# BloodAxe/segmentation-networks-benchmark

Hardware: AMD Instinct MI355X
Metric: images/sec/GPU (fwd+bwd) ZF_UNET 224x224 bs=32; 1/2/4/8-GPU scaling (higher is better)
Workload: dtype bf16; 1 GPU; ZF_UNET 224x224 bf16 bs=32/GPU, bce_dice, SGD lr 1e-3, Dropout2d 0.2, train step torch_train.py:180-190 (configs[1]); global_batch=32, parallelism=dp1

## Files before the change

segmentation-networks-benchmark_amd/csrc/common.h:

```cpp
#pragma once
#include <hip/hip_runtime.h>
#include <hip/hip_ext.h>
#include <stdint.h>
#include <stdio.h>
#include <string.h>

#include "../../include/segnb_hip.h"

typedef __attribute__((ext_vector_type(8))) __bf16 bf16x8_t;
typedef __attribute__((ext_vector_type(16))) float f32x16_t;

struct bf16_t {
    unsigned short bits;
};

void segnb_set_error(const char* fmt, ...);

#define SEGNB_CHECK_ARG_AS(who, cond, msg)                           \
    do {                                                             \
        if (!(cond)) {                                               \
            segnb_set_error("%s: bad argument: %s", who, msg);       \
            return SEGNB_E_BADARG;                                   \
        }                                                            \
    } while (0)
// ... 73 lines not shown
    if (plan_scope__.top && g_segnb_census_on) segnb_census(#fn);                            \
    if (plan_scope__.top && segnb_plan_recording()) segnb_plan_record_call(#fn, fn, __VA_ARGS__)
void segnb_plan_refuse(const char* why);
#define SEGNB_PLAN_REFUSE(why)                                         \
    SegnbPlanScope plan_scope__;                                       \
    if (plan_scope__.top && g_segnb_census_on) segnb_census(__func__); \
    if (plan_scope__.top && segnb_plan_recording()) segnb_plan_refuse(why)

int segnb_num_cus();
bool segnb_fprop_general_forced();
int segnb_knob_fprop_dma();
int segnb_knob_fprop_dma_cfg();
int segnb_knob_fprop_dma_dbg();
int segnb_knob_fprop_nostats();
int segnb_knob_rw_store_waves();
int segnb_knob_bnreduce_fused();
int segnb_knob_fprop_deepk();
int segnb_knob_fprop_thin();
enum segnb_try_outcome {
    SEGNB_TRY_DECLINED = 0,
    SEGNB_TRY_LAUNCHED,
    SEGNB_TRY_DELIVERED,
};
inline int segnb_try_launched(segnb_try_outcome* did, int rc) {
    if (rc == 0) *did = SEGNB_TRY_LAUNCHED;
    return rc;
}
inline void segnb_kernel_took(segnb_try_outcome did, const char** served, const char* name) {
    if (did != SEGNB_TRY_DECLINED && *served == nullptr) *served = name;
}
template <class Args>
__attribute__((always_inline)) inline bool take_bn_reduce(Args& a, const segnb_conv_geom* g, const segnb_bn_reduce_epilogue* bn) {
    const long long yb = (((long long)g->N * g->Ho * g->Wo - 1) * bn->ld_y + g->Co) * 2;
    if (yb >= (1ll << 31)) return false;
    a.bn_y = (const bf16_t*)bn->y;
    a.bn_y_bytes = (unsigned)yb;
    a.bn_ld = bn->ld_y;
    a.bn_coef = bn->coef;
    a.bn_sums = bn->sums;
    a.bn_act = bn->act;
    a.bn_slope = bn->slope;
    return true;
}
template <class Args>
__attribute__((always_inline)) inline void take_act_epilogue(Args& a, const segnb_act_epilogue* ep) {
    a.ep_act = ep != nullptr ? ep->act : -1;
    a.ep_coef = ep != nullptr ? ep->coef : nullptr;
    a.ep_slope = ep != nullptr ? ep->slope : 0.f;
}
int segnb_fprop_thin_try(segnb_try_outcome* did, const segnb_conv_geom* g, const void* in, const void* wpacked, void* out,
                         hipStream_t stream, const segnb_bn_reduce_epilogue* bn);
int segnb_fprop_thin_ok(const segnb_conv_geom* g);
int segnb_knob_fprop_upd();
int segnb_knob_fprop_drop();
int segnb_knob_fprop_mask();
int segnb_fprop_dma_actmask_ok(const segnb_conv_geom* g);
int segnb_fprop_roll_actmask_ok(const segnb_conv_geom* g);
int segnb_knob_fprop_mf16();
int segnb_knob_fprop_rw();
int segnb_knob_fprop_ksplit();
float* segnb_head_scratch(size_t bytes, hipStream_t stream);
void segnb_head_bwd_finish(const float* part, int gx, int gy, int K, int C, int CT, float* dw, float* db, hipStream_t stream);
int segnb_knob_pack_blocks();
int segnb_knob_fprop_roll();
int segnb_knob_wg_cu_pct();
int segnb_knob_conv_cus();
int segnb_fprop_dma_read_stamps(unsigned long long* host_dst);
int segnb_fprop_s1_try(segnb_try_outcome* did, const segnb_conv_geom* g, const void* in, const void* wpacked, const float* bias, int bias_n,
                       void* out, double* stats, hipStream_t stream, const float* drop = nullptr, int ld_drop = 0, int stats_ld = 0);
int segnb_fprop_dma_try(segnb_try_outcome* did, const segnb_conv_geom* g, const void* in, unsigned in_bytes, const void* wpacked,
                        unsigned w_bytes, const float* bias, int bias_n, void* out, double* stats,
                        hipStream_t stream, const segnb_act_epilogue* ep = nullptr, const segnb_upcat_src* uc = nullptr,
                        const segnb_bn_reduce_epilogue* bn = nullptr);
int segnb_fprop_rw_try(segnb_try_outcome* did, const segnb_conv_geom* g, const void* in, unsigned in_bytes, const void* wpacked,
                       unsigned w_bytes, const float* bias, int bias_n, void* out, double* stats,
                       hipStream_t stream, const segnb_bn_reduce_epilogue* bn = nullptr,
                       const segnb_act_epilogue* ep = nullptr, const segnb_upcat_src* uc = nullptr,
                       const segnb_upcat_src* upsum = nullptr);
int segnb_fprop_roll_try(segnb_try_outcome* did, const segnb_conv_geom* g, const void* in, unsigned in_bytes, const void* wpacked,
                         unsigned w_bytes, const float* bias, int bias_n, void* out, double* stats, hipStream_t stream,
                         const segnb_bn_reduce_epilogue* bn = nullptr, const segnb_operand_tf* tf = nullptr,
                         const segnb_upcat_src* uc = nullptr);
int segnb_fprop_c8_try(segnb_try_outcome* did, const segnb_conv_geom* g, const void* in, const void* wpacked, const float* bias, int bias_n,
                       void* out, double* stats, hipStream_t stream, const segnb_act_epilogue* ep = nullptr);
struct segnb_wgrad_bnapply {
    const void* g;
    int ld_g;
    const void* y;
    int ld_y;
    const float* coef;
    const float* bcoef;
    int Cp;
    int act;
    float slope;
};
int segnb_wgrad_s1_try(segnb_try_outcome* did, const segnb_conv_geom* g, const void* in, const void* dout, float* dwp, int nslab,
                       hipStream_t stream, bool partial, const segnb_wgrad_bnapply* bna = nullptr,
                       const segnb_upcat_src* uc = nullptr, const segnb_wgrad_target* tgt = nullptr);
const segnb_wgrad_target* segnb_take_wgrad_target();
void segnb_wgrad_to_param(float* dwp, int Cop, int ntaps, int Cip, int nslab, const segnb_wgrad_target* tgt, bool rezero,
                          hipStream_t stream);
int segnb_wgrad_s1_slabs(const segnb_conv_geom* g);
void segnb_slab_reduce(float* dwp, long long total, int nslab, hipStream_t stream);
bool segnb_wgrad_roll_applies(const segnb_conv_geom* g);
int segnb_wgrad_roll_try(segnb_try_outcome* did, const segnb_conv_geom* g, const void* in, const void* dout, float* dwp, int nslab,
                         hipStream_t stream, bool partial, const segnb_operand_tf* tfx = nullptr, const segnb_operand_tf* tfd = nullptr);
// ... 137 lines not shown
```

segmentation-networks-benchmark_amd/csrc/fprop_dma.hip:

```cpp
#include "common.h"

#include "fprop_dma.h"

#include <mutex>
#include <vector>

#ifndef SEGNB_EXP
#define SEGNB_EXP 0
#endif

namespace {

__device__ unsigned long long g_stamps[3 * 256 * 4];
#define FD_STAMP(role, step, k)                                                                      \
    do {                                                                                            \
        if (DBG && ((a.dbg & 32) || ((a.dbg & 64) && (role) == 0 && (k) == 0)) && blockIdx.x == 0 && lane == 0 &&  \
            (step) < 256)                                                                            \
            g_stamps[((role) * 256 + (step)) * 4 + (k)] = __builtin_amdgcn_s_memtime();             \
    } while (0)

template <int BN_, int R_, int WT_, int CW_M_, bool TALL_ = false, bool MF16_ = true, int NTAP_ = 9, int UP_ = 0>
struct WsCfg {
    static constexpr bool UPD_ = UP_ == 1;
    static constexpr bool UPF = UP_ == 2;
    static_assert(UP_ == 0 || (NTAP_ == 4 && !TALL_ && MF16_), "up-sampled segment forms: 2 x 2 window, 16x16x32 form");
    static constexpr int BN = BN_, R = R_, WT = WT_;
    static constexpr int NTAP = NTAP_, KW = NTAP_ == 9 ? 3 : 2, KH = KW;
    static constexpr bool UPD = UPD_;
    static constexpr int UP = UP_;
    static constexpr int NPL = UPD_ ? 4 : 1;
    static_assert(NTAP_ == 9 || NTAP_ == 4, "3 x 3 or 2 x 2 tap window");
    static_assert(!UPD_ || (NTAP_ == 4 && !TALL_ && MF16_), "plane gather: 2 x 2 window, 16x16x32 form");
    static constexpr bool TALL = TALL_;
    static constexpr bool MF16 = MF16_;
    static constexpr int BM = TALL_ ? 256 : (R_ * WT_ + 16 * CW_M_ - 1) / (16 * CW_M_) * (16 * CW_M_);
    static constexpr int TM16 = BM / CW_M_ / 16, TN16 = BN_ / (4 / CW_M_) / 16;
    static constexpr int NB = 4;
    static constexpr int NT = 512, NCW = 4, NLW = 4;
    static_assert(R * WT <= BM, "tile pixels");
    static constexpr int NRD = TM16 + TN16, NMF = TM16 * TN16;
    static constexpr int rd_before(int q) { return (q * NRD + NMF - 1) / NMF; }
    static constexpr int WAVES_M = CW_M_, WAVES_N = NCW / CW_M_;
    static constexpr int WM = BM / WAVES_M, WN = BN / WAVES_N;
    static constexpr int TM = WM / 32, TN = WN / 32;
    static constexpr int XR = R + KH - 1, XC = WT + 2, NPIX = XR * XC;
    static constexpr int APIECES = (NPIX + 7) / 8;
    static constexpr int A_BYTES = APIECES * 1024;
    static constexpr int NBW = 2, NAW = 2;
    static constexpr int APW = (APIECES + NAW - 1) / NAW;
    static constexpr int A_STEPS = NTAP - 2;
    static constexpr int APS = (APW + A_STEPS - 1) / A_STEPS;
    static constexpr int BPIECES = BN / 8;
    static constexpr int B_STAGE = BN * 128;
    static constexpr int BPW = BPIECES / NBW;
    static constexpr int OUT_ROW = BN * 2 + 16;
    static constexpr int OC = BN / 8;
    static constexpr int MT = NCW * 64;
    static constexpr int RPT = BM / (MT / OC);
    static constexpr int OFF_B = 2 * A_BYTES;
    static constexpr int OFF_STG = OFF_B + NB * B_STAGE;
    static constexpr int OFF_DUMMY = OFF_STG + BM * OUT_ROW;
    static constexpr int OFF_PIX = OFF_DUMMY + 1024;
    static constexpr int OFF_BIAS = OFF_PIX + 4 * BM * 4;
    static constexpr int OFF_SCALE = OFF_BIAS + BN * 4;
    static constexpr int OFF_TICKET = OFF_SCALE + BN * 4;
    static constexpr int SMEM = OFF_TICKET + 16;
    static constexpr int RED_BYTES = MT * 16 * 8;
    static_assert(WM % (MF16_ ? 16 : 32) == 0 && WN % (MF16_ ? 16 : 32) == 0 && WAVES_M * WAVES_N == NCW, "wave tiling");
    static_assert(BPIECES % NBW == 0 && NBW + NAW == NLW, "fetch wave roles");
    static_assert(MT % OC == 0 && MT >= 2 * BN && RPT <= 8 && BM <= MT && BM % (MT / OC) == 0, "store pass / statistics threads");
    static constexpr bool MASK_OK = MF16_ && !TALL_ && BM == 256 && CW_M_ == 4 && SMEM + 2048 <= 160 * 1024;
    static_assert(RED_BYTES <= OFF_STG, "statistics reduction scratch");
    static_assert(SMEM <= 160 * 1024, "LDS");
    static_assert(TM + TN <= 6, "fragment wait statement");
};

template <class C, bool DBG, bool EP = false, bool STATS = true, bool SPLITK = false, bool MASK = false>
__global__ __launch_bounds__(512) void conv_fprop_ws_kernel(const FdArgs a) {
    static_assert(!SPLITK || (!EP && !DBG && C::UP == 0 && C::NTAP == 9), "split K: plain 3 x 3 forward / data gradient");
    static_assert(!MASK || (STATS && !EP && !DBG && !SPLITK && C::MF16 && C::UP == 0 && C::NTAP == 9 && !C::TALL && C::BM == 256 &&
                            C::BN == 64 && C::WAVES_M == 4 && C::SMEM + 2048 <= 160 * 1024),
                  "activation mask: plain 3 x 3 data gradient, 16x16x32 form, 256 x 64 tiles, 2 KB of mask bytes behind the LDS layout");
    constexpr int BN = C::BN, R = C::R, WT = C::WT, BM = C::BM, TM = C::TM, TN = C::TN, XC = C::XC;
    constexpr int NT = C::NT, NB = C::NB, APW = C::APW, APS = C::APS, BPW = C::BPW, OC = C::OC, NLW = C::NLW;
    constexpr int OUT_ROW = C::OUT_ROW, NF = TM + TN;
    constexpr int NTAP = C::NTAP, KW = C::KW;
    constexpr int SM = NTAP & 3;

    extern __shared__ __attribute__((aligned(1024))) unsigned char smem[];
    int* sPix = reinterpret_cast<int*>(smem + C::OFF_PIX);
    float* sBias = reinterpret_cast<float*>(smem + C::OFF_BIAS);
    const unsigned lds0 = (unsigned)(size_t)smem;

    const int tid = threadIdx.x, lane = tid & 63, wave = __builtin_amdgcn_readfirstlane(tid >> 6);
    const int r = lane & 31, h = lane >> 5;
    const bool loader = wave >= C::NCW;
    const int lw = wave - C::NCW;
    const int wm = (wave & 3) / C::WAVES_N, wn = (wave & 3) % C::WAVES_N;
// ... 92 lines not shown
                        return;
                    }
                    const int pl = c / a.NCHP, sl = c - pl * a.NCHP;
                    const int t16 = (2 * (t >> 1) - (pl >> 1) + 1) * 4 + (2 * (t & 1) - (pl & 1) + 1);
                    soff = (unsigned)(t16 * a.Ci + sl * 64) * 2u;
                } else if constexpr (C::UPF) {
                    soff = (unsigned)((3 - t) * a.Ci + c * 64) * 2u;
                } else {
                    soff = (unsigned)(t * a.Ci + (c + c_off) * 64) * 2u;
                }
        #pragma unroll
                for (int pb = 0; pb < BPW; ++pb)
                    dma16(lds0 + C::OFF_B + stage * C::B_STAGE + ((lw & 1) * BPW + pb) * 1024, b_voff[pb], rs_w, soff);
            };

            fetch_b(0, 0, 0);
            fetch_b(0, 1, 1);
            fetch_b(0, 2, 2);
            asm volatile("s_waitcnt vmcnt(0)" ::: "memory");
            lds_barrier();
            for (; it < a.IT; it += a.GM) {
                for (int c = 0; c < a.NCH; ++c, ++cg) {
                    const int cn = c + 1 == a.NCH ? 0 : c + 1;
                    static_for<NTAP>([&](auto t_c) {
                        constexpr int t = decltype(t_c)::value;
                        constexpr int tf = t + 3 < NTAP ? t + 3 : t + 3 - NTAP;
                        const int cf = t + 3 < NTAP ? c : cn;
                        if (lw == 0) FD_STAMP(1, cg * 9 + t, 0);
                        if (!(SEGNB_EXP & 1) && !(DBG && (a.dbg & 1))) fetch_b(cf, tf, (cg * SM + t + 3) & (NB - 1));
                        if (lw == 0) FD_STAMP(1, cg * 9 + t, 1);
                        asm volatile("s_waitcnt vmcnt(%0)" ::"n"(BPW) : "memory");
                        if (lw == 0) FD_STAMP(1, cg * 9 + t, 2);
                        if (!(SEGNB_EXP & 64) || t % 3 == 2) raw_barrier();
                        if (lw == 0) FD_STAMP(1, cg * 9 + t, 3);
                    });
                }
            }
        } else {
            unsigned a_rel[APW], a_xy[APW], a_voff[C::NPL][APW];
            unsigned a_uoff[APW];
            const bool vcat = a.u != nullptr;
        #pragma unroll
            for (int pa = 0; pa < APW; ++pa) {
                const int pix = ((lw & 1) + C::NAW * pa) * 8 + (lane >> 3);
                const int q = lane & 7;
                const int xr = pix / XC, xc = pix - xr * XC;
                const int key = C::XC % 2 == 0 ? xc : pix;
                a_rel[pa] = (unsigned)((xr * a.Wi + xc) * (C::UPD ? 2 : 1)) * (unsigned)a.ld_x * 2u +
                            (unsigned)((q ^ ((key >> 1) & 7)) * 16);
                if constexpr (C::UPD)
                    if (a.P32)
                        a_rel[pa] = (unsigned)((xr * a.Wi + xc) * 2) * (unsigned)a.ld_x * 2u + (unsigned)(((q ^ ((key >> 1) & 7)) & 3) * 16);
                a_xy[pa] = pix < C::NPIX ? (unsigned)xr | ((unsigned)xc << 16) : 0x7fff7fffu;
            }
            auto set_fetch_tile = [&](int it, int table) {
                const bool live = it < a.IT;
                if constexpr (C::TALL) {
                    const int HV = a.H + 1, VT = a.N * HV;
                    const float inv = 1.0f / (float)HV;
                    const int v0 = it * R + a.dhmin;
        #pragma unroll
                    for (int pa = 0; pa < APW; ++pa) {
                        const int v = v0 + (int)(a_xy[pa] & 0xffffu), wi = a.dwmin + (int)(a_xy[pa] >> 16);
                        const int n = (int)(((float)v + 0.5f) * inv);
                        const int hh = v - n * HV;
                        const bool ok = live && (unsigned)v < (unsigned)VT && hh < a.H && (unsigned)wi < (unsigned)a.Wi;
                        const int pix = ((lw & 1) + C::NAW * pa) * 8 + (lane >> 3);
                        a_voff[0][pa] = ok ? (unsigned)((n * a.Hi + hh) * a.Wi + wi) * (unsigned)a.ld_x * 2u +
                                              (unsigned)(((lane & 7) ^ ((pix >> 1) & 7)) * 16)
                                        : OOB;
                    }
                    const int t128 = (lw & 1) * 64 + lane;
        #pragma unroll
                    for (int rr = t128; rr < BM; rr += C::NAW * 64) {
                        const int v = it * R + rr / WT, wo = rr % WT;
                        const int n = (int)(((float)v + 0.5f) * inv);
                        const int hh = v - n * HV;
                        sPix[table * BM + rr] =
                            (live && rr < R * WT && v < VT && hh < a.H && wo < a.W) ? (n * a.H + hh) * a.W + wo : -1;
                    }
                    return;
                }
                const int n = it / (a.HB * a.WB);
                const int rem = it - n * (a.HB * a.WB);
                const int hb = rem / a.WB, wb = rem - hb * a.WB;
                if constexpr (C::UPD) {
                    const unsigned hlim = live ? (unsigned)a.H : 0u;
                    static_for<4>([&](auto pl_c) {
                        constexpr int pl = decltype(pl_c)::value, py = pl >> 1, px = pl & 1;
                        const int y0 = hb * R - py, x0 = wb * WT - px;
                        const unsigned base = (unsigned)(((n * a.Hi + 2 * y0 + py) * a.Wi + 2 * x0 + px) * a.ld_x * 2);
        #pragma unroll
                        for (int pa = 0; pa < APW; ++pa) {
                            const int yp = y0 + (int)(a_xy[pa] & 0xffffu), xp = x0 + (int)(a_xy[pa] >> 16);
                            const bool ok = (unsigned)yp < hlim && (unsigned)xp < (unsigned)a.W;
                            a_voff[pl][pa] = ok ? base + a_rel[pa] : OOB;
                        }
                    });
                    if (a.P32) {
        #pragma unroll
                        for (int pa = 0; pa < APW; ++pa) {
                            const int xc = (int)(a_xy[pa] >> 16);
                            const bool second = ((((int)lane & 7) ^ ((xc >> 1) & 7)) >> 2) != 0;
                            a_voff[0][pa] = second ? a_voff[1][pa] : a_voff[0][pa];
                            a_voff[1][pa] = second ? a_voff[3][pa] : a_voff[2][pa];
                        }
                    }
                } else {
                const int h0 = hb * R + (C::UPF ? py - 1 : a.dhmin), w0 = wb * WT + (C::UPF ? px - 1 : a.dwmin);
                const unsigned base = (unsigned)(((n * a.Hi + h0) * a.Wi + w0) * a.ld_x * 2);
                const unsigned hlim = live ? (unsigned)a.Hi : 0u;
        #pragma unroll
                for (int pa = 0; pa < APW; ++pa) {
                    const int hi = h0 + (int)(a_xy[pa] & 0xffffu), wi = w0 + (int)(a_xy[pa] >> 16);
                    const bool ok = (unsigned)hi < hlim && (unsigned)wi < (unsigned)a.Wi;
                    a_voff[0][pa] = ok ? base + a_rel[pa] : OOB;
                    if (vcat) {
                        const int pixl = ((lw & 1) + C::NAW * pa) * 8 + (lane >> 3);
                        const int keyl = C::XC % 2 == 0 ? pixl % XC : pixl;
                        a_uoff[pa] = ok ? (unsigned)((n * a.Hu + (hi >> 1)) * a.Wu + (wi >> 1)) * (unsigned)a.ld_u * 2u +
                                              (unsigned)(((lane & 7) ^ ((keyl >> 1) & 7)) * 16)
                                        : OOB;
                    }
                }
                }
                const int t128 = (lw & 1) * 64 + lane;
        #pragma unroll
                for (int rr = t128; rr < BM; rr += C::NAW * 64) {
                    const int ho = hb * R + rr / WT, wo = wb * WT + rr % WT;
                    const bool in_tile = R * WT == BM || rr < R * WT;
                    if constexpr (C::UPF)
                        sPix[table * BM + rr] = (live && ho < a.H && wo < a.W) ? (n * 2 * a.H + 2 * ho + py) * (2 * a.W) + 2 * wo + px : -1;
                    else
                        sPix[table * BM + rr] = (live && in_tile && ho < a.H && wo < a.W) ? (n * a.H + ho) * a.W + wo : -1;
                }
            };
            auto fetch_a = [&](int p0, int p1, int c_, int buf) {
                const int c = c_ + c_off;
                int pl = 0;
                unsigned soff = (unsigned)c * 128u;
                if constexpr (C::UPD) {
                    if (a.P32) {
                        pl = c;
                        soff = 0u;
                    } else {
                        pl = c / a.NCHP;
                        soff = (unsigned)(c - pl * a.NCHP) * 128u;
                    }
                }
                if constexpr (!C::UPD && !C::UPF && !C::TALL) {
                    if (vcat) {
                        if (c < a.NCHU) {
        #pragma unroll
                            for (int pa = 0; pa < APW; ++pa) {
                                if (pa >= p0 && pa < p1) {
                                    const int piece = (lw & 1) + C::NAW * pa;
                                    const unsigned dst = piece < C::APIECES ? lds0 + buf * C::A_BYTES + piece * 1024 : lds0 + C::OFF_DUMMY;
                                    dma16(dst, a_uoff[pa], rs_u, (unsigned)c * 128u);
                                }
                            }
                            return;
                        }
                        soff = (unsigned)(c - a.NCHU) * 128u;
                    }
                }
                auto go = [&](auto pl_c) {
                    constexpr int PL = decltype(pl_c)::value;
        #pragma unroll
                    for (int pa = 0; pa < APW; ++pa) {
                        if (pa >= p0 && pa < p1) {
                            const int piece = (lw & 1) + C::NAW * pa;
                            const unsigned dst = piece < C::APIECES ? lds0 + buf * C::A_BYTES + piece * 1024 : lds0 + C::OFF_DUMMY;
                            dma16(dst, a_voff[PL][pa], rs_x, soff);
                        }
                    }
                };
                if constexpr (C::UPD) {
                    if (pl == 0) go(std::integral_constant<int, 0>{});
                    else if (pl == 1) go(std::integral_constant<int, 1>{});
                    else if (pl == 2) go(std::integral_constant<int, 2>{});
                    else go(std::integral_constant<int, 3>{});
                } else {
                    go(std::integral_constant<int, 0>{});
                }
// ... 50 lines not shown
                            if (!(SEGNB_EXP & 2) && !(DBG && (a.dbg & 2))) fetch_a(t * APS, (t + 1) * APS, cn, abuf ^ 1);
                        if constexpr (MASK) {
                            if constexpr (t == 0)
                                if (c == 0) mask_request(tile_no & 3);
                            if constexpr (t == NTAP - 1)
                                if (last) mask_publish();
                        }
                        if constexpr (t == NTAP - 2)
                            if (next_last) set_fetch_tile(setup_it, setup_tab);
                        if (lw == C::NBW) FD_STAMP(2, cg * 9 + t, 1);
                        if constexpr (t == NTAP - 2) {
                            asm volatile("s_waitcnt vmcnt(0)" ::: "memory");
                        }
                        if (lw == C::NBW) FD_STAMP(2, cg * 9 + t, 2);
                        if (!(SEGNB_EXP & 64) || t % 3 == 2) raw_barrier();
                        if (lw == C::NBW) FD_STAMP(2, cg * 9 + t, 3);
                    });
                }
            }
        }
        asm volatile("s_waitcnt vmcnt(0)" ::: "memory");
        if constexpr (SPLITK) {
            raw_barrier();
            raw_barrier();
        }
        raw_barrier();
        raw_barrier();
        raw_barrier();
    } else {
        constexpr bool MF16 = C::MF16;
        int tile_no_out = 0;
        bool pending_out = false;
        constexpr int TM16 = C::TM16, TN16 = C::TN16;
        int b_rd[MF16 ? 1 : TN];
        int a_rd[MF16 ? 1 : 9][MF16 ? 1 : TM];
        static_assert(!MF16 || XC % 2 == 0, "16x16x32 form: the swizzle key must be the halo column");
        int b_rd16[MF16 ? 2 : 1][MF16 ? TN16 : 1];
        int a_rd16[MF16 ? KW : 1][MF16 ? TM16 : 1][MF16 ? 2 : 1];
        if constexpr (MF16) {
            const int r16 = lane & 15, g4 = lane >> 4;
    #pragma unroll
            for (int j = 0; j < TN16; ++j) {
                const int row = wn * C::WN + 16 * j + r16;
                const int v = C::OFF_B + row * 128 + ((g4 ^ ((row >> 1) & 7)) << 4);
                b_rd16[0][j] = v;
                b_rd16[1][j] = v ^ 64;
            }
    #pragma unroll
            for (int dwi = 0; dwi < KW; ++dwi)
    #pragma unroll
                for (int i = 0; i < TM16; ++i) {
                    const int m_ = wm * C::WM + 16 * i + r16;
                    const int m = (R * WT == BM || m_ < R * WT) ? m_ : 0;
                    const int p = (m / WT) * XC + (m % WT) + a.dw[dwi];
                    const int key = p % XC;
                    int v = (p << 7) + ((g4 ^ ((key >> 1) & 7)) << 4);
                    asm volatile("" : "+v"(v));
                    a_rd16[dwi][i][0] = v;
                    a_rd16[dwi][i][1] = v ^ 64;
                }
        } else {
        #pragma unroll
            for (int j = 0; j < TN; ++j) {
                const int row = wn * C::WN + 32 * j + r;
                b_rd[j] = C::OFF_B + row * 128 + ((row & 12) << 3) + (((h ^ (row >> 1)) & 1) << 4);
            }
        #pragma unroll
            for (int t = 0; t < 9; ++t)
        #pragma unroll
                for (int i = 0; i < TM; ++i) {
                    const int m = wm * C::WM + 32 * i + r;
                    const int p = (m / WT) * XC + (m % WT) + a.dh[t] * XC + a.dw[t];
                const int key = XC % 2 == 0 ? p % XC : p;
                int v = (p << 7) + ((key & 12) << 3) + (((h ^ (key >> 1)) & 1) << 4);
                    asm volatile("" : "+v"(v));
                    a_rd[t][i] = v;
                }

        }
        lds_barrier();
        unsigned char* const sOut = smem + C::OFF_STG;
        const __amdgpu_buffer_rsrc_t rs_out = make_rsrc(a.out, a.out_bytes);
        const int cc = tid % OC, row0 = tid / OC;
        const bool cok = n_base + cc * 8 < a.Co;
        float s1[8], s2[8];
#pragma unroll
        for (int e = 0; e < 8; ++e) s1[e] = s2[e] = 0.f;
        int row_pix = -1, row_pix2 = -1;
        u32x4_t row_v = {0, 0, 0, 0}, row_v2 = {0, 0, 0, 0};
        constexpr bool T14 = !C::TALL && R * WT != BM;
        static_assert(!T14 || (R == 14 && WT == 14 && C::MT / OC == 32 && C::RPT == 7), "store rows of the 14 x 14 tile");
        const bool row_live = !T14 || (row0 & 15) < WT;
        const int row_first = !T14 ? row0 : (row_live ? (row0 >> 4) * WT + (row0 & 15) : R * WT);
        const int row_step = !T14 ? C::MT / OC : (row_live ? 2 * WT : 0);
        auto row_load = [&](int k, const int* tab) {
            const int row = row_first + k * row_step;
            const unsigned a_pix = (unsigned)(size_t)(tab + row), a_v = (unsigned)(size_t)(sOut + row * OUT_ROW + cc * 16);
            asm volatile("ds_read_b32 %0, %1" : "=v"(row_pix) : "v"(a_pix));
            asm volatile("ds_read_b128 %0, %1" : "=v"(row_v) : "v"(a_v));
        };
        auto row_load2 = [&](int k, const int* tab) {
            const int row = row_first + k * row_step;
            const unsigned a_pix = (unsigned)(size_t)(tab + row), a_v = (unsigned)(size_t)(sOut + row * OUT_ROW + cc * 16);
            asm volatile("ds_read_b32 %0, %1" : "=v"(row_pix2) : "v"(a_pix));
            asm volatile("ds_read_b128 %0, %1" : "=v"(row_v2) : "v"(a_v));
        };
        auto row_store_of = [&](int opix, const u32x4_t v) {
// ... 559 lines not shown
    return 0;
}

using WsCfg14 = WsCfg<64, 14, 14, 2, false, true>;

bool ws14_serves(const FdArgs& a) {
    return a.H % 14 == 0 && a.W % 14 == 0 && a.W <= 56 && a.Co > 32 && a.bn_y == nullptr && a.ep_act < 0 && !a.dbg &&
           a.up_out == nullptr && segnb_knob_fprop_mf16();
}

int launch_ws14(FdArgs& a, hipStream_t stream) {
    using C = WsCfg14;
    static int attr_rc = [] {
        hipError_t e = hipFuncSetAttribute(reinterpret_cast<const void*>(conv_fprop_ws_kernel<C, false>),
                                           hipFuncAttributeMaxDynamicSharedMemorySize, C::SMEM);
        if (e == hipSuccess)
            e = hipFuncSetAttribute(reinterpret_cast<const void*>(conv_fprop_ws_kernel<C, false, false, false>),
                                    hipFuncAttributeMaxDynamicSharedMemorySize, C::SMEM);
        if (e != hipSuccess) segnb_set_error("fprop_ws hipFuncSetAttribute: %s", hipGetErrorString(e));
        return (int)e;
    }();
    if (attr_rc) return attr_rc;
    a.HB = a.H / C::R;
    a.WB = a.W / C::WT;
    a.IT = a.N * a.HB * a.WB;
    a.NTL = (a.Co + C::BN - 1) / C::BN;
    a.NCH = a.Ci / 64;
    a.KS = 1;
    a.ntmajor = 0;
    int gm = segnb_knob_conv_cus() / a.NTL;
    if (gm < 1) gm = 1;
    if (gm > a.IT) gm = a.IT;
    a.GM = gm;
    if (g_segnb_census_on) segnb_census("tile:ws14");
    if (a.stats == nullptr && segnb_knob_fprop_nostats())
        hipLaunchKernelGGL((conv_fprop_ws_kernel<C, false, false, false>), dim3(a.GM * a.NTL), dim3(C::NT), C::SMEM, stream, a);
    else
        hipLaunchKernelGGL((conv_fprop_ws_kernel<C, false>), dim3(a.GM * a.NTL), dim3(C::NT), C::SMEM, stream, a);
    return 0;
}

template <class C>
int launch_ws_upd(FdArgs& a, hipStream_t stream) {
    static int attr_rc = [] {
        hipError_t e = hipFuncSetAttribute(reinterpret_cast<const void*>(conv_fprop_ws_kernel<C, false, false, false>),
                                           hipFuncAttributeMaxDynamicSharedMemorySize, C::SMEM);
        if (e != hipSuccess) segnb_set_error("fprop_ws hipFuncSetAttribute: %s", hipGetErrorString(e));
        return (int)e;
    }();
    if (attr_rc) return attr_rc;
    a.HB = (a.H + C::R - 1) / C::R;
    a.WB = (a.W + C::WT - 1) / C::WT;
    a.IT = a.N * a.HB * a.WB;
    a.NTL = (a.Co + C::BN - 1) / C::BN;
    a.P32 = a.Ci == 32;
    a.NCHP = a.P32 ? 1 : a.Ci / 64;
    a.NCH = a.P32 ? 2 : 4 * a.NCHP;
    a.RPS = a.NCH * C::NTAP - 1 < C::RPT ? 2 : 1;
    if ((a.NCH * C::NTAP - 1) * a.RPS < C::RPT) return NOT_HANDLED;
    int gm = segnb_knob_conv_cus() / a.NTL;
    if (gm < 1) gm = 1;
    if (gm > a.IT) gm = a.IT;
    a.GM = gm;
    hipLaunchKernelGGL((conv_fprop_ws_kernel<C, false, false, false>), dim3(a.GM * a.NTL), dim3(C::NT), C::SMEM, stream, a);
    return 0;
}

template <class C>
int launch_ws_upf(FdArgs& a, hipStream_t stream) {
    static int attr_rc = [] {
        hipError_t e = hipFuncSetAttribute(reinterpret_cast<const void*>(conv_fprop_ws_kernel<C, false, false, true>),
                                           hipFuncAttributeMaxDynamicSharedMemorySize, C::SMEM);
        if (e != hipSuccess) segnb_set_error("fprop_ws hipFuncSetAttribute: %s", hipGetErrorString(e));
        return (int)e;
    }();
    if (attr_rc) return attr_rc;
    a.HB = (a.H + C::R - 1) / C::R;
    a.WB = (a.W + C::WT - 1) / C::WT;
    a.IT = a.N * a.HB * a.WB;
    a.NTLR = (a.Co + C::BN - 1) / C::BN;
    a.NTL = 4 * a.NTLR;
    a.NCH = a.Ci / 64;
    a.NCHP = a.NCH;
    a.P32 = 0;
    a.RPS = a.NCH * C::NTAP - 1 < C::RPT ? 2 : 1;
    if ((a.NCH * C::NTAP - 1) * a.RPS < C::RPT) return NOT_HANDLED;
    int gm = segnb_knob_conv_cus() / a.NTL;
    if (gm < 1) gm = 1;
    if (gm > a.IT) gm = a.IT;
    a.GM = gm;
    hipLaunchKernelGGL((conv_fprop_ws_kernel<C, false, false, true>), dim3(a.GM * a.NTL), dim3(C::NT), C::SMEM, stream, a);
    return 0;
}

bool upd_geometry(const segnb_conv_geom* g) {
    if (g->ntaps != 16 || g->in_step != 2 || g->out_step != 1 || g->oh0 != 0 || g->ow0 != 0) return false;
    if (g->QH != g->Ho || g->QW != g->Wo || g->Hi != 2 * g->Ho || g->Wi != 2 * g->Wo) return false;
    if ((g->Ci % 64 != 0 && g->Ci != 32) || g->Co <= 32 || g->Wo < 12) return false;
    for (int t = 0; t < 16; ++t)
        if (g->dh[t] != t / 4 - 1 || g->dw[t] != t % 4 - 1) return false;
    return true;
}

int try_upd(const segnb_conv_geom* g, FdArgs& a, hipStream_t stream) {
    if (!upd_geometry(g)) return NOT_HANDLED;
    a.Ktot = 16 * g->Ci;
    a.dhmin = a.dwmin = 0;
    for (int t = 0; t < 9; ++t) a.dh[t] = a.dw[t] = 0;
    a.dh[2] = a.dh[3] = 1;
    a.dw[1] = a.dw[3] = 1;
    const int ntl = (g->Co + 63) / 64;
    int gm = segnb_knob_conv_cus() / ntl;
    if (gm < 1) gm = 1;
    const long long it0 = (long long)g->N * ((g->Ho + 7) / 8) * ((g->Wo + 31) / 32);
    const long long it1 = (long long)g->N * ((g->Ho + 15) / 16) * ((g->Wo + 15) / 16);
    int cfg = segnb_knob_fprop_dma_cfg();
    if (cfg < 0) cfg = (it0 + gm - 1) / gm < (it1 + gm - 1) / gm ? 0 : 1;
    if (cfg == 0) return launch_ws_upd<WsCfg<64, 8, 32, 4, false, true, 4, 1>>(a, stream);
    return launch_ws_upd<WsCfg<64, 16, 16, 4, false, true, 4, 1>>(a, stream);
}

constexpr unsigned WS14_DEFAULT_LEVELS = 7u;

int dispatch_fd(FdArgs& a, hipStream_t stream) {
    int cfg = segnb_knob_fprop_dma_cfg();
    bool row_major_taps = true;
    for (int t = 0; t < 9; ++t) row_major_taps = row_major_taps && a.dw[t] == a.dw[t % 3] && a.dh[t] == a.dh[3 * (t / 3)];
    const bool can14 = row_major_taps && ws14_serves(a);
    if (cfg == 3 && !can14) cfg = -1;
    if (cfg < 0) {
        if (a.Co <= 32) return NOT_HANDLED;
        if (a.W <= 8) {
            if (a.W != 7 || a.H != 7) return NOT_HANDLED;
            return launch_ws<WsCfg<64, 36, 7, 4, true, false>>(a, stream);
        }
        const int ntl = (a.Co + 63) / 64;
        int gm = segnb_knob_conv_cus() / ntl;
        if (gm < 1) gm = 1;
        const long long it0 = (long long)a.N * ((a.H + 7) / 8) * ((a.W + 31) / 32);
        const long long it1 = (long long)a.N * ((a.H + 15) / 16) * ((a.W + 15) / 16);
        const long long r0 = (it0 + gm - 1) / gm, r1 = (it1 + gm - 1) / gm;
        cfg = r0 < r1 ? 0 : 1;
        if (a.bn_y != nullptr) cfg = 1;
        const bool same_stats = a.stats == nullptr || a.W == 14;
        if (can14 && same_stats && a.H == a.W && ((a.W == 14 && (WS14_DEFAULT_LEVELS & 1u)) || (a.W == 28 && (WS14_DEFAULT_LEVELS & 2u)) ||
                                                  (a.W == 56 && (WS14_DEFAULT_LEVELS & 4u)))) {
            const long long it3 = (long long)a.N * (a.H / 14) * (a.W / 14);
            const long long r3 = (it3 + gm - 1) / gm;
            if (r3 * WsCfg14::BM < (cfg == 0 ? r0 : r1) * 256) cfg = 3;
        }
    }
    if (cfg == 3) return launch_ws14(a, stream);
    if (segnb_knob_fprop_mf16() && row_major_taps) {
        switch (cfg) {
            case 0: return launch_ws<WsCfg<64, 8, 32, 4, false, true>>(a, stream);
            case 1: return launch_ws<WsCfg<64, 16, 16, 4, false, true>>(a, stream);
            case 2: return launch_ws<WsCfg<64, 36, 7, 4, true, false>>(a, stream);
            default: return NOT_HANDLED;
        }
    }
    switch (cfg) {
        case 0: return launch_ws<WsCfg<64, 8, 32, 4, false, false>>(a, stream);
        case 1: return launch_ws<WsCfg<64, 16, 16, 4, false, false>>(a, stream);
        case 2: return launch_ws<WsCfg<64, 36, 7, 4, true, false>>(a, stream);
        default: return NOT_HANDLED;
    }
}

}

// ... 177 lines not shown
```

segmentation-networks-benchmark_amd/csrc/runtime.hip:

```cpp
#include <stdarg.h>
#include <stdlib.h>

#include "common.h"

static thread_local char g_err[512] = "";

void segnb_set_error(const char* fmt, ...) {
    va_list ap;
    va_start(ap, fmt);
    vsnprintf(g_err, sizeof(g_err), fmt, ap);
    va_end(ap);
}

int segnb_num_cus() {
    static int cus = 0;
    if (cus > 0) return cus;
    int dev = 0;
    hipDeviceProp_t prop;
    if (hipGetDevice(&dev) != hipSuccess || hipGetDeviceProperties(&prop, dev) != hipSuccess) return 256;
    cus = prop.multiProcessorCount > 0 ? prop.multiProcessorCount : 256;
    return cus;
}

extern "C" const char* segnb_last_error(void) { return g_err; }
// ... 220 lines not shown
    }
    return g_fprop_dma_cfg;
}
static int g_fprop_rw = 1;
int segnb_knob_fprop_rw() { return g_fprop_rw && segnb_knob_fprop_dma_cfg() < 0; }
static int g_fprop_roll = -2;
int segnb_knob_fprop_roll() {
    if (g_fprop_roll == -2) {
        const char* e = getenv("SEGNB_FPROP_ROLL");
        g_fprop_roll = e != nullptr ? atoi(e) : 2;
    }
    return segnb_knob_fprop_dma() ? g_fprop_roll : 0;
}
static int g_pack_blocks = 0;
int segnb_knob_pack_blocks() { return g_pack_blocks; }

static int g_wgrad_roll = 0;
int segnb_knob_wgrad_roll() { return g_wgrad_roll; }
static int g_wgrad_c8roll = 1;
int segnb_knob_wgrad_c8roll() { return g_wgrad_c8roll; }
static int g_conv_cu_pct = 100;
int segnb_knob_conv_cus() {
    const int n = segnb_num_cus() * g_conv_cu_pct / 100;
    return n < 1 ? 1 : n;
}
static int g_wg_cu_pct = 0;
int segnb_knob_wg_cu_pct() { return g_wg_cu_pct; }
static int g_fprop_deepk = -2;
int segnb_knob_fprop_deepk() {
    if (g_fprop_deepk == -2) {
        const char* e = getenv("SEGNB_FPROP_DEEPK");
        g_fprop_deepk = (e != nullptr && e[0] == '0') ? 0 : 1;
    }
    return g_fprop_deepk;
}
static int g_fprop_thin = 1;
int segnb_knob_fprop_thin() { return g_fprop_thin; }
static int g_fprop_mf16 = -2;
int segnb_knob_fprop_mf16() {
    if (g_fprop_mf16 == -2) {
        const char* e = getenv("SEGNB_FPROP_MF16");
        g_fprop_mf16 = (e != nullptr && e[0] == '0') ? 0 : 1;
    }
    return g_fprop_mf16;
}
static int g_fprop_upd = -2;
int segnb_knob_fprop_upd() {
    if (g_fprop_upd == -2) {
        const char* e = getenv("SEGNB_FPROP_UPD");
        g_fprop_upd = (e != nullptr && e[0] == '0') ? 0 : 1;
    }
    return g_fprop_upd;
}
static int g_fprop_mask = -2;
int segnb_knob_fprop_mask() {
    if (g_fprop_mask == -2) {
        const char* e = getenv("SEGNB_FPROP_MASK");
        g_fprop_mask = (e != nullptr && e[0] == '0') ? 0 : 1;
    }
    return g_fprop_mask;
}
static int g_fprop_drop = -2;
int segnb_knob_fprop_drop() {
    if (g_fprop_drop == -2) {
        const char* e = getenv("SEGNB_FPROP_DROP");
        g_fprop_drop = (e != nullptr && e[0] == '0') ? 0 : 1;
    }
    return g_fprop_drop;
}
static int g_fprop_nostats = 1;
int segnb_knob_fprop_nostats() { return g_fprop_nostats; }
static int g_rw_store_waves = 4;
int segnb_knob_rw_store_waves() { return g_rw_store_waves; }
static int g_bnreduce_fused = -2;
int segnb_knob_bnreduce_fused() {
    if (g_bnreduce_fused == -2) {
        const char* e = getenv("SEGNB_BNREDUCE_FUSED");
        g_bnreduce_fused = (e != nullptr && e[0] == '0') ? 0 : 1;
    }
    return g_bnreduce_fused;
}
static int g_fprop_ksplit = -2;
int segnb_knob_fprop_ksplit() {
    if (g_fprop_ksplit == -2) {
        const char* e = getenv("SEGNB_FPROP_KSPLIT");
        g_fprop_ksplit = e != nullptr ? atoi(e) : 1;
    }
    return g_fprop_ksplit;
}
static int g_fprop_dma_dbg = 0;
int segnb_knob_fprop_dma_dbg() { return g_fprop_dma_dbg; }
extern "C" int segnb_wg_cu_share(int pct) {
    SEGNB_PLAN_RECORD(segnb_wg_cu_share, pct);
    g_wg_cu_pct = pct < 0 ? 0 : (pct > 100 ? 100 : pct);
    return 0;
}

static thread_local segnb_wgrad_target g_wg_target;
static thread_local bool g_wg_target_armed = false;
extern "C" int segnb_wgrad_target_arm(const segnb_wgrad_target* t) {
    SEGNB_PLAN_RECORD(segnb_wgrad_target_arm, t);
    SEGNB_CHECK_ARG(t != nullptr && t->gw != nullptr, "NULL target");
    SEGNB_CHECK_ARG(t->ntaps >= 1 && t->ntaps <= SEGNB_MAX_TAPS && t->Ci > 0 && t->Co > 0 && t->s_in >= t->ntaps && t->ci_off >= 0 &&
                        t->s_out >= (long long)(t->ci_off + t->Ci) * t->s_in, "bad target layout");
    for (int i = 0; i < t->ntaps; ++i) SEGNB_CHECK_ARG(t->kpos[i] >= 0 && t->kpos[i] < t->s_in, "bad kernel position");
    g_wg_target = *t;
// ... 28 lines not shown
    if (strcmp(key, "wgrad_roll") == 0) {
        g_wgrad_roll = value ? 1 : 0;
        return 0;
    }
    if (strcmp(key, "wgrad_c8roll") == 0) {
        g_wgrad_c8roll = value ? 1 : 0;
        return 0;
    }
    if (strcmp(key, "fprop_rw") == 0) {
        g_fprop_rw = value ? 1 : 0;
        return 0;
    }
    if (strcmp(key, "conv_cu_pct") == 0) {
        g_conv_cu_pct = value < 1 ? 1 : (value > 100 ? 100 : value);
        return 0;
    }
    if (strcmp(key, "plan_profile") == 0) {
        if (value == 2) plan_profile_dump();
        else g_plan_profile = value;
        return 0;
    }
    if (strcmp(key, "wg_cu_pct") == 0) {
        g_wg_cu_pct = value < 0 ? 0 : (value > 100 ? 100 : value);
        return 0;
    }
    if (strcmp(key, "fprop_drop") == 0) {
        g_fprop_drop = value ? 1 : 0;
        return 0;
    }
    if (strcmp(key, "fprop_mask") == 0) {
        g_fprop_mask = value ? 1 : 0;
        return 0;
    }
    if (strcmp(key, "fprop_nostats") == 0) {
        g_fprop_nostats = value ? 1 : 0;
        return 0;
    }
    if (strcmp(key, "rw_store_waves") == 0) {
        g_rw_store_waves = value == 2 ? 2 : (value == 8 ? 8 : 4);
        return 0;
    }
    if (strcmp(key, "bnreduce_fused") == 0) {
        g_bnreduce_fused = value ? 1 : 0;
        return 0;
    }
    if (strcmp(key, "fprop_deepk") == 0) {
        g_fprop_deepk = value ? 1 : 0;
        return 0;
    }
    if (strcmp(key, "fprop_thin") == 0) {
        g_fprop_thin = value ? 1 : 0;
        return 0;
    }
    if (strcmp(key, "fprop_mf16") == 0) {
        g_fprop_mf16 = value ? 1 : 0;
        return 0;
    }
    if (strcmp(key, "call_census") == 0) {
        g_segnb_census_on = value ? 1 : 0;
        return 0;
    }
    if (strcmp(key, "fprop_ksplit") == 0) {
        g_fprop_ksplit = value < 0 ? 0 : value;
        return 0;
    }
    if (strcmp(key, "fprop_dma_dbg") == 0) {
        g_fprop_dma_dbg = value;
        return 0;
    }
    segnb_set_error("segnb_tune: unknown key '%s'", key);
    return SEGNB_E_BADARG;
}

extern "C" int segnb_debug_stamps(unsigned long long* host_dst) {
    SEGNB_CHECK_ARG(host_dst != nullptr, "NULL destination");
    return segnb_fprop_dma_read_stamps(host_dst);
}
```

Baseline: 6805 images/s.

## Add 14x14 tile and four-image 7x7 packing for upsample-gather convolutions

Extends the plane-gather upsampled conv path with two new tile forms. A 14x14 tile serves 14/28/56 outputs when a cost estimate favours it over the 256-row tiles. A Q4 form packs four 7x7 images into one 196-row tile so the 7x7 decoder layer uses the custom kernel instead of falling back. Both aim to cut padded or wasted rows in the MFMA tiles and the number of passes per CU. In exchange they add index arithmetic in the address setup, per-image bounds masks and more template instantiations.

```diff
diff --git a/segmentation-networks-benchmark_amd/csrc/common.h b/segmentation-networks-benchmark_amd/csrc/common.h
--- a/segmentation-networks-benchmark_amd/csrc/common.h
+++ b/segmentation-networks-benchmark_amd/csrc/common.h
@@ -149,6 +149,8 @@
                          hipStream_t stream, const segnb_bn_reduce_epilogue* bn);
 int segnb_fprop_thin_ok(const segnb_conv_geom* g);
 int segnb_knob_fprop_upd();
+int segnb_knob_fprop_up7();
+int segnb_knob_fprop_up14();
 int segnb_knob_fprop_drop();
 int segnb_knob_fprop_mask();
 int segnb_fprop_dma_actmask_ok(const segnb_conv_geom* g);
diff --git a/segmentation-networks-benchmark_amd/csrc/fprop_dma.hip b/segmentation-networks-benchmark_amd/csrc/fprop_dma.hip
--- a/segmentation-networks-benchmark_amd/csrc/fprop_dma.hip
+++ b/segmentation-networks-benchmark_amd/csrc/fprop_dma.hip
@@ -19,8 +19,10 @@
             g_stamps[((role) * 256 + (step)) * 4 + (k)] = __builtin_amdgcn_s_memtime();             \
     } while (0)
 
-template <int BN_, int R_, int WT_, int CW_M_, bool TALL_ = false, bool MF16_ = true, int NTAP_ = 9, int UP_ = 0>
+template <int BN_, int R_, int WT_, int CW_M_, bool TALL_ = false, bool MF16_ = true, int NTAP_ = 9, int UP_ = 0, bool Q4_ = false>
 struct WsCfg {
+    static constexpr bool Q4 = Q4_;
+    static_assert(!Q4_ || (UP_ == 1 && R_ == 14 && WT_ == 14 && CW_M_ == 2), "four 7 x 7 images per tile: plane gather on the 224-row form");
     static constexpr bool UPD_ = UP_ == 1;
     static constexpr bool UPF = UP_ == 2;
     static_assert(UP_ == 0 || (NTAP_ == 4 && !TALL_ && MF16_), "up-sampled segment forms: 2 x 2 window, 16x16x32 form");
@@ -43,7 +45,7 @@
     static constexpr int WAVES_M = CW_M_, WAVES_N = NCW / CW_M_;
     static constexpr int WM = BM / WAVES_M, WN = BN / WAVES_N;
     static constexpr int TM = WM / 32, TN = WN / 32;
-    static constexpr int XR = R + KH - 1, XC = WT + 2, NPIX = XR * XC;
+    static constexpr int XR = Q4_ ? 16 : R + KH - 1, XC = WT + 2, NPIX = XR * XC;
     static constexpr int APIECES = (NPIX + 7) / 8;
     static constexpr int A_BYTES = APIECES * 1024;
     static constexpr int NBW = 2, NAW = 2;
@@ -242,6 +244,11 @@
                     if (a.P32)
                         a_rel[pa] = (unsigned)((xr * a.Wi + xc) * 2) * (unsigned)a.ld_x * 2u + (unsigned)(((q ^ ((key >> 1) & 7)) & 3) * 16);
                 a_xy[pa] = pix < C::NPIX ? (unsigned)xr | ((unsigned)xc << 16) : 0x7fff7fffu;
+                if constexpr (C::Q4) {
+                    const int qi = (xr >> 3) * 2 + (xc >> 3), ly = xr & 7, lx = xc & 7;
+                    a_rel[pa] = (unsigned)(((qi * a.Hi + 2 * ly) * a.Wi + 2 * lx) * a.ld_x * 2) + (unsigned)((q ^ ((key >> 1) & 7)) * 16);
+                    a_xy[pa] = (unsigned)ly | ((unsigned)lx << 16);
+                }
             }
             auto set_fetch_tile = [&](int it, int table) {
                 const bool live = it < a.IT;
@@ -271,8 +278,8 @@
                     }
                     return;
                 }
-                const int n = it / (a.HB * a.WB);
-                const int rem = it - n * (a.HB * a.WB);
+                const int n = C::Q4 ? 4 * it : it / (a.HB * a.WB);
+                const int rem = C::Q4 ? 0 : it - n * (a.HB * a.WB);
                 const int hb = rem / a.WB, wb = rem - hb * a.WB;
                 if constexpr (C::UPD) {
                     const unsigned hlim = live ? (unsigned)a.H : 0u;
@@ -283,7 +290,11 @@
         #pragma unroll
                         for (int pa = 0; pa < APW; ++pa) {
                             const int yp = y0 + (int)(a_xy[pa] & 0xffffu), xp = x0 + (int)(a_xy[pa] >> 16);
-                            const bool ok = (unsigned)yp < hlim && (unsigned)xp < (unsigned)a.W;
+                            bool ok = (unsigned)yp < hlim && (unsigned)xp < (unsigned)a.W;
+                            if constexpr (C::Q4) {
+                                const int pix = ((lw & 1) + C::NAW * pa) * 8 + (lane >> 3);
+                                ok = ok && n + (pix / XC >> 3) * 2 + (pix % XC >> 3) < a.N;
+                            }
                             a_voff[pl][pa] = ok ? base + a_rel[pa] : OOB;
                         }
                     });
@@ -319,7 +330,9 @@
                 for (int rr = t128; rr < BM; rr += C::NAW * 64) {
                     const int ho = hb * R + rr / WT, wo = wb * WT + rr % WT;
                     const bool in_tile = R * WT == BM || rr < R * WT;
-                    if constexpr (C::UPF)
+                    if constexpr (C::Q4)
+                        sPix[table * BM + rr] = (live && in_tile && n + rr / 49 < a.N) ? n * 49 + rr : -1;
+                    else if constexpr (C::UPF)
                         sPix[table * BM + rr] = (live && ho < a.H && wo < a.W) ? (n * 2 * a.H + 2 * ho + py) * (2 * a.W) + 2 * wo + px : -1;
                     else
                         sPix[table * BM + rr] = (live && in_tile && ho < a.H && wo < a.W) ? (n * a.H + ho) * a.W + wo : -1;
@@ -476,7 +489,11 @@
                 for (int i = 0; i < TM16; ++i) {
                     const int m_ = wm * C::WM + 16 * i + r16;
                     const int m = (R * WT == BM || m_ < R * WT) ? m_ : 0;
-                    const int p = (m / WT) * XC + (m % WT) + a.dw[dwi];
+                    int p = (m / WT) * XC + (m % WT) + a.dw[dwi];
+                    if constexpr (C::Q4) {
+                        const int qi = m / 49, rem = m - qi * 49;
+                        p = ((qi >> 1) * 8 + rem / 7) * XC + (qi & 1) * 8 + rem % 7 + a.dw[dwi];
+                    }
                     const int key = p % XC;
                     int v = (p << 7) + ((g4 ^ ((key >> 1) & 7)) << 4);
                     asm volatile("" : "+v"(v));
@@ -1142,6 +1159,11 @@
     a.HB = (a.H + C::R - 1) / C::R;
     a.WB = (a.W + C::WT - 1) / C::WT;
     a.IT = a.N * a.HB * a.WB;
+    if constexpr (C::Q4) {
+        if (a.H != 7 || a.W != 7 || a.Ci % 64 != 0) return NOT_HANDLED;
+        a.HB = a.WB = 1;
+        a.IT = (a.N + 3) / 4;
+    }
     a.NTL = (a.Co + C::BN - 1) / C::BN;
     a.P32 = a.Ci == 32;
     a.NCHP = a.P32 ? 1 : a.Ci / 64;
@@ -1152,6 +1174,7 @@
     if (gm < 1) gm = 1;
     if (gm > a.IT) gm = a.IT;
     a.GM = gm;
+    if (g_segnb_census_on && C::BM != 256) segnb_census(C::Q4 ? "tile:up7" : "tile:up14");
     hipLaunchKernelGGL((conv_fprop_ws_kernel<C, false, false, false>), dim3(a.GM * a.NTL), dim3(C::NT), C::SMEM, stream, a);
     return 0;
 }
@@ -1186,7 +1209,8 @@
 bool upd_geometry(const segnb_conv_geom* g) {
     if (g->ntaps != 16 || g->in_step != 2 || g->out_step != 1 || g->oh0 != 0 || g->ow0 != 0) return false;
     if (g->QH != g->Ho || g->QW != g->Wo || g->Hi != 2 * g->Ho || g->Wi != 2 * g->Wo) return false;
-    if ((g->Ci % 64 != 0 && g->Ci != 32) || g->Co <= 32 || g->Wo < 12) return false;
+    if ((g->Ci % 64 != 0 && g->Ci != 32) || g->Co <= 32) return false;
+    if (g->Wo < 12 && !(g->Wo == 7 && g->Ho == 7 && g->Ci % 64 == 0 && segnb_knob_fprop_up7())) return false;
     for (int t = 0; t < 16; ++t)
         if (g->dh[t] != t / 4 - 1 || g->dw[t] != t % 4 - 1) return false;
     return true;
@@ -1199,13 +1223,25 @@
     for (int t = 0; t < 9; ++t) a.dh[t] = a.dw[t] = 0;
     a.dh[2] = a.dh[3] = 1;
     a.dw[1] = a.dw[3] = 1;
+    if (g->Wo < 12) return launch_ws_upd<WsCfg<64, 14, 14, 2, false, true, 4, 1, true>>(a, stream);
     const int ntl = (g->Co + 63) / 64;
     int gm = segnb_knob_conv_cus() / ntl;
     if (gm < 1) gm = 1;
     const long long it0 = (long long)g->N * ((g->Ho + 7) / 8) * ((g->Wo + 31) / 32);
     const long long it1 = (long long)g->N * ((g->Ho + 15) / 16) * ((g->Wo + 15) / 16);
+    const long long r0 = (it0 + gm - 1) / gm, r1 = (it1 + gm - 1) / gm;
+    const bool can14 = g->Ho % 14 == 0 && g->Wo % 14 == 0 && g->Ci % 64 == 0;
     int cfg = segnb_knob_fprop_dma_cfg();
-    if (cfg < 0) cfg = (it0 + gm - 1) / gm < (it1 + gm - 1) / gm ? 0 : 1;
+    if (cfg == 3 && !can14) cfg = -1;
+    if (cfg < 0) {
+        cfg = r0 < r1 ? 0 : 1;
+        if (can14 && segnb_knob_fprop_up14() && g->Ho == g->Wo && (g->Wo == 14 || g->Wo == 28 || g->Wo == 56)) {
+            const long long it3 = (long long)g->N * (g->Ho / 14) * (g->Wo / 14);
+            const long long r3 = (it3 + gm - 1) / gm;
+            if (r3 * WsCfg14::BM < (cfg == 0 ? r0 : r1) * 256) cfg = 3;
+        }
+    }
+    if (cfg == 3) return launch_ws_upd<WsCfg<64, 14, 14, 2, false, true, 4, 1>>(a, stream);
     if (cfg == 0) return launch_ws_upd<WsCfg<64, 8, 32, 4, false, true, 4, 1>>(a, stream);
     return launch_ws_upd<WsCfg<64, 16, 16, 4, false, true, 4, 1>>(a, stream);
 }
diff --git a/segmentation-networks-benchmark_amd/csrc/runtime.hip b/segmentation-networks-benchmark_amd/csrc/runtime.hip
--- a/segmentation-networks-benchmark_amd/csrc/runtime.hip
+++ b/segmentation-networks-benchmark_amd/csrc/runtime.hip
@@ -296,6 +296,22 @@
     }
     return g_fprop_upd;
 }
+static int g_fprop_up7 = -2;
+int segnb_knob_fprop_up7() {
+    if (g_fprop_up7 == -2) {
+        const char* e = getenv("SEGNB_FPROP_UP7");
+        g_fprop_up7 = (e != nullptr && e[0] == '0') ? 0 : 1;
+    }
+    return g_fprop_up7;
+}
+static int g_fprop_up14 = -2;
+int segnb_knob_fprop_up14() {
+    if (g_fprop_up14 == -2) {
+        const char* e = getenv("SEGNB_FPROP_UP14");
+        g_fprop_up14 = (e != nullptr && e[0] == '0') ? 0 : 1;
+    }
+    return g_fprop_up14;
+}
 static int g_fprop_mask = -2;
 int segnb_knob_fprop_mask() {
     if (g_fprop_mask == -2) {
@@ -430,6 +446,14 @@
         g_fprop_thin = value ? 1 : 0;
         return 0;
     }
+    if (strcmp(key, "fprop_up7") == 0) {
+        g_fprop_up7 = value ? 1 : 0;
+        return 0;
+    }
+    if (strcmp(key, "fprop_up14") == 0) {
+        g_fprop_up14 = value ? 1 : 0;
+        return 0;
+    }
     if (strcmp(key, "fprop_mf16") == 0) {
         g_fprop_mf16 = value ? 1 : 0;
         return 0;
```

After: 6828 images/s, median of 6. About the same (+0.3%).
